# OxfordML/GPz

Measured on AMD Instinct MI355X. Metric: objective+gradient evals/sec, higher is better.
Workload: dtype f64

## Files before the change

### gpz_amd/csrc/gpz_ctx.h

```cpp
#pragma once
#include <hip/hip_runtime.h>
#include <math.h>
#include <stdarg.h>
#include <stdio.h>
#include <stdlib.h>
#include <string.h>
#include <algorithm>
#include <atomic>
#include <mutex>
#include <string>
#include <type_traits>
#include <vector>
#include "../../include/gpz_hip.h"
#include "gpz_dev.h"
#include "gpz_kernels.h"
#include <map>

#define HIPCHK(x)                                                                                   \
    do {                                                                                            \
        hipError_t e_ = (x);                                                                        \
        if (e_ != hipSuccess) return gpz_fail(GPZ_ERR_HIP, "%s:%d %s: %s", __FILE__, __LINE__, #x, hipGetErrorString(e_)); \
    } while (0)

inline int method_id_of(const char *m) {
// ... 173 lines not shown
    int nchunk = 1, rows_per_chunk = 1;
    int tile_rows = 0, ntiles = 1, tile_nchunk = 1, tile_rpc = 1;
    double *tile_rstats = nullptr;
    double *partial = nullptr, *rstats = nullptr, *dGfull = nullptr, *spart = nullptr;
    double *nupart = nullptr, *rowscal = nullptr, *frec = nullptr;
    bool syrk_small = false;
    bool small_tail_dp = false;
    bool small_tail = false;
    int st_nwg = 0, st_nf = 0;
    bool mom_ring = false;
    int mom_nv = 0;
    double *st_slab = nullptr;
    bool fused = true;
    double *phipart = nullptr;
    int phipart_groups = 0;
    long phipart_rows = 0;
    int nslots = 0;
    double *out_d = nullptr;
    double *out_h = nullptr, *theta_h = nullptr;
    gpz_allreduce_fn ar_fn = nullptr;
    void *ar_user = nullptr;
    void *priv = nullptr;
    void (*priv_free)(void *) = nullptr;
    int timing = 0;
    bool time_rest = false;
    struct GraphSeg {
        hipGraphExec_t exec = nullptr;
        int stage = -1;
        bool count_call = false;
        double *hook_buf = nullptr;
// ... 100 lines not shown
```

### gpz_amd/csrc/gpz_ctx.hip

```cpp
#include "gpz_ctx.h"

namespace gpzi {
static int upload_rowset(gpz_ctx *c, RowSet &rs, int64_t n_tot, const double *X, const double *Y, const double *omega,
                         const uint8_t *mask, bool need_xr, const double *Psi = nullptr) {
    const int d = c->d, de = c->de, k = c->k;
    std::vector<int64_t> idx;
    idx.reserve((size_t)n_tot);
    for (int64_t i = 0; i < n_tot; ++i)
        if (!mask || mask[i]) idx.push_back(i);
    if (c->gen) {
        std::vector<int> hg0(idx.size());
        for (size_t r = 0; r < idx.size(); ++r) {
            std::vector<unsigned char> pt(d);
            for (int c_ = 0; c_ < d; ++c_) { const double xv = X[(size_t)c_ * n_tot + idx[r]]; pt[c_] = (xv != xv) ? 0 : 1; }
            int g = -1;
            for (size_t q = 0; q < c->pats.size(); ++q)
                if (c->pats[q] == pt) { g = (int)q; break; }
            if (g < 0) {
                if (c->pats_fixed) return gpz_fail(GPZ_ERR_ARG, "row %lld has a NaN pattern that is not in the given pattern table", (long long)idx[r]);
                c->pats.push_back(pt);
                g = (int)c->pats.size() - 1;
            }
            hg0[r] = g;
        }
// ... 380 lines not shown
        if ((rc = c->ar.alloc(&c->fin_part, (size_t)c->ngroups * c->m * (c->d + c->d * c->d + 2)))) return bail(rc);
        if (!c->has_psi) {
            const int nmt = c->de + c->de * (c->de + 1) / 2;
            c->gen_tnch = 2048 / ((c->m + 255) / 256);
            if (c->gen_tnch < 1) c->gen_tnch = 1;
            if ((rc = build_chunks(c->gen_tnch, 32))) return bail(rc);
            const size_t nslab = c->mom_nchunk > 0 ? (size_t)c->mom_nchunk : 1;
            if ((rc = c->ar.alloc(&c->gen_tslab, nslab * c->m * (nmt + 2)))) return bail(rc);
            if ((rc = c->ar.alloc(&c->gen_frec, (size_t)c->ngroups * c->m * (nmt + 2)))) return bail(rc);
        }
        if (c->va.n_pad && (rc = c->ar.alloc(&c->Phi_v, (size_t)c->va.n_pad * c->mp))) return bail(rc);
    }
    if ((rc = alloc_mm(c))) return bail(rc);

    const size_t np = c->tr.n_pad, mp = c->mp, k = c->k, m = c->m;
    {
        size_t want = c->opt.row_tile > 0 ? (size_t)c->opt.row_tile : 0;
        size_t fr = 0, tot = 0;
        if (!want && hipMemGetInfo(&fr, &tot) == hipSuccess) {
            DevCache &dc = dev_cache();
            std::lock_guard<std::mutex> g(dc.mu);
            auto it = dc.held.find(c->device);
            if (it != dc.held.end()) fr += it->second;
        }
        if (!want && fr && 2.0 * (double)np * (double)mp * 8.0 > 0.7 * (double)fr) {
            want = (size_t)(0.35 * (double)fr / (2.0 * (double)mp * 8.0));
            if (want < 131072) want = 131072;
        }
        const bool can = !c->gen;
        if (want && can) {
            const size_t tr = (size_t)rup((long)want, 1024);
            if (tr < np) {
                c->tile_rows = (int)tr;
                c->ntiles = (int)((np + tr - 1) / tr);
            }
        }
    }
    const size_t npt = c->tile_rows ? (size_t)c->tile_rows : np;
    if ((rc = c->ar.alloc(&c->Phi, npt * mp))) return bail(rc);
    c->small_tail = !c->gen && !c->has_psi && !c->tile_rows &&
                    small_tail_fits(c->kind, c->de, c->m, k, c->mp, c->has_missing) && !c->opt.small_tail_off;
// ... 58 lines not shown
        c->rows_per_split = rup((int)((np_k + s1 - 1) / s1), 16);
        c->nsplit = (int)((np_k + c->rows_per_split - 1) / c->rows_per_split);
        c->rows_per_split_d = rup((int)((np_k + s2 - 1) / s2), 16);
        c->nsplit_d = (int)((np_k + c->rows_per_split_d - 1) / c->rows_per_split_d);
        size_t need = (size_t)(c->nsplit > c->nsplit_d ? c->nsplit : c->nsplit_d) * mp * mp;
        c->syrk_small = syrk_small_fits(mp) && !c->psi32 && !c->opt.syrk_small_off;
        if (c->syrk_small) {
            const size_t ns = syrk_small_slab_count((int)np_k, mp);
            if (ns > need) need = ns;
        }
        size_t need_l = (size_t)c->nsplit_l * c->mq * c->mq;
        c->slab_count = need > need_l ? need : need_l;
        if ((rc = c->ar.alloc(&c->slab, c->slab_count))) return bail(rc);
    }
    {
        size_t prow = npt < 1024 * 1024 ? npt : 0;
        if (c->va.n_pad && (size_t)c->va.n_pad < 1024 * 1024 && (size_t)c->va.n_pad > prow) prow = (size_t)c->va.n_pad;
        if (prow) {
            c->phipart_groups = 16;
            c->phipart_rows = (long)prow;
            if ((rc = c->ar.alloc(&c->phipart, (size_t)c->phipart_groups * 2 * k * prow))) return bail(rc);
        }
    }
    c->comm1_count = k * mp * mp + gpz_ns(c->k);
    if ((rc = c->ar.alloc(&c->comm1, c->comm1_count))) return bail(rc);
    c->comm2_count = m * c->nm + k * 2 * mp + k * 4 + gpz_ns(c->k);
    if ((rc = c->ar.alloc(&c->comm2, c->comm2_count))) return bail(rc);
    c->nwg_rows = c->tr.n < 2048 ? (c->tr.n > 0 ? c->tr.n : 1) : 2048;
    if (!c->fused) {
        if ((rc = c->ar.alloc(&c->colslab, (size_t)c->nwg_rows * 2 * mp))) return bail(rc);
        if ((rc = c->ar.alloc(&c->scal_slab, (size_t)c->nwg_rows * 4))) return bail(rc);
    } else {
        c->nslots = gpz_gemm_wave_cols() * ((c->mp + 127) / 128);
        if ((rc = c->ar.alloc(&c->nupart, (size_t)c->nslots * npt))) return bail(rc);
        if ((rc = c->ar.alloc(&c->rowscal, (size_t)4 * np))) return bail(rc);
        if ((rc = c->ar.alloc(&c->frec, (size_t)m * (c->nm + 2)))) return bail(rc);
// ... 159 lines not shown
    if (f32req && !c->psi32)
        why = !c->gen || !c->has_psi ? " [dtype f32 requested: no input noise on a covariance kind, nothing runs in fp32]"
              : c->d > 20            ? " [dtype f32 requested: d > 20 has no fp32 pair kernel, fp64 route]"
                                     : " [dtype f32 requested: rows with missing dimensions, fp64 route]";
    const int gstate = c->gset[c->timing == 2 ? 1 : 0].state;
    const size_t nseg = c->gset[c->timing == 2 ? 1 : 0].segs.size();
    char gsb[96];
    if (gstate == 2 && nseg > 1) snprintf(gsb, sizeof gsb, "replayed (%zu segments%s)", nseg, c->desc.world > 1 ? ", all-reduce between them" : "");
    else snprintf(gsb, sizeof gsb, "%s", gstate == 2 ? "replayed" : gstate == -1 ? "disabled (recording failed)" : c->opt.no_graph ? "disabled (GPZ_NO_GRAPH)"
                                         : c->timing == 1 ? "off (stage timing on)" : "eager (not recorded yet)");
    const char *gs = gsb;
    const bool f32mm = c->psi32 && !c->opt.f32_contractions_off;
    char rows[96];
    if (c->tile_rows) snprintf(rows, sizeof rows, "; rows: streamed, %d tiles of %d (PHI built twice per evaluation)", c->ntiles, c->tile_rows);
    else rows[0] = 0;
    return snprintf(buf, (size_t)cap, "pair/PHI kernels: %s%s; contractions: %s MFMA%s%s; evaluation graph: %s%s%s", phi, why,
                    f32mm ? "fp32-operand (fp64 master sums)" : "fp64",
                    c->syrk_small ? ", PHI' W PHI with the whole triangle in one workgroup (k_syrk_small)" : "",
                    c->small_tail ? ", T-GEMM + row scalars + moments in one kernel (k_small_tail: T stays in registers)" :
                    c->small_tail_dp ? ", T-GEMM + row scalars + dPHI in one kernel (k_small_tail; moment sums with input noise by k_moments_diag)" : "", gs, rows,
                    c->mom_ring ? "; moments: k_moments_ring (PHI, T through an LDS ring)" : "");
}
namespace gpzi {

}
```

### gpz_amd/csrc/gpz_eval.hip

```cpp
#include "gpz_ctx.h"

namespace gpzi {
static GenRows gen_rows(const RowSet &rs) {
    GenRows r{};
    r.Xr = rs.Xr; r.gid = rs.gid; r.Psi3 = rs.Psi3; r.rows_by_group = rs.rows_by_group; r.n = rs.n; r.n_pad = rs.n_pad;
    return r;
}

static void psi32_chunks(const gpz_ctx *c, int *nch, int *rpc) {
    int r = (c->tr.n + c->gen_nchunk - 1) / c->gen_nchunk;
    r = rup(r > 0 ? r : 1, 64);
    *rpc = r;
    *nch = c->tr.n > 0 ? (c->tr.n + r - 1) / r : 1;
}

static int allreduce(gpz_ctx *c, double *buf, size_t count) {
    if (c->desc.world <= 1) return 0;
    if (!c->ar_fn) return gpz_fail(GPZ_ERR_COMM, "world=%d but no all-reduce hook set (gpz_ctx_set_allreduce)", c->desc.world);
    if (c->capturing) {
        if (graph_cut(c)) return gpz_fail(GPZ_ERR_HIP, "evaluation graph: cut at an exchange point failed");
        c->cap->segs.back().hook_buf = buf;
        c->cap->segs.back().hook_count = count;
        return 0;
    }
// ... 115 lines not shown
            launch_gen_phi(c->st, gen_rows(c->tr), c->m, c->mp, c->d, c->de, c->k, c->pr.P, c->Sig, c->lnS, c->pat_d,
                           c->Phi, c->tr.Y, c->gen_ws);
        }
        launch_gen_rowdot(c->st, c->Phi, c->mp, c->tr.n, c->tr.n_pad, c->m, c->k, c->hetero ? c->pr.v : nullptr, c->pr.b,
                          c->tr.om, nullptr, c->lnbeta, c->wbeta, nullptr, c->tr.om_ld);
    } else {
        Stage s(c, "phi_build");
        PhiArgs a{};
        a.Xc = c->tr.Xc; a.ldx = c->tr.n_pad; a.n = c->tr.n; a.n_pad = c->tr.n_pad;
        a.m = c->m; a.mp = c->mp; a.d = c->de; a.k = c->k; a.kind = c->kind;
        a.P = c->pr.P; a.G = (c->kind == GPZ_KIND_COV) ? c->pr.Rc : c->pr.G2;
        a.v = c->hetero ? c->pr.v : nullptr; a.b = c->pr.b; a.omega = c->tr.om; a.om_ld = c->tr.om_ld; a.Y = c->tr.Y;
        a.Phi = c->Phi; a.lnbeta = c->lnbeta; a.wbeta = c->wbeta; a.w = nullptr; a.phiw = nullptr;
        a.Psic = c->tr.Psic; a.Mc = c->tr.Mc; a.ucnt = c->tr.ucnt;
        a.part = a.n_pad <= c->phipart_rows ? c->phipart : nullptr; a.part_groups = c->phipart_groups;
        if (launch_phi(c->st, a)) return gpz_fail(GPZ_ERR_UNSUPPORTED, "PHI kernel not instantiated for d=%d", c->de);
    }
    return 0;
}

struct RowTile { long r0; int rows, rows_pad; };
static RowTile row_tile(const gpz_ctx *c, int t) {
    RowTile rt;
    rt.r0 = (long)t * c->tile_rows;
    const long left_pad = (long)c->tr.n_pad - rt.r0, left = (long)c->tr.n - rt.r0;
    rt.rows_pad = (int)(left_pad < c->tile_rows ? left_pad : c->tile_rows);
    rt.rows = (int)(left < 0 ? 0 : (left < rt.rows_pad ? left : rt.rows_pad));
    return rt;
}
static int phi_tile(gpz_ctx *c, const RowTile &rt) {
    PhiArgs a{};
    const long r0 = rt.r0;
    a.Xc = c->tr.Xc + r0; a.ldx = c->tr.n_pad; a.n = rt.rows; a.n_pad = rt.rows_pad;
    a.m = c->m; a.mp = c->mp; a.d = c->de; a.k = c->k; a.kind = c->kind;
    a.P = c->pr.P; a.G = (c->kind == GPZ_KIND_COV) ? c->pr.Rc : c->pr.G2;
    a.v = c->hetero ? c->pr.v : nullptr; a.b = c->pr.b; a.omega = c->tr.om ? c->tr.om + r0 : nullptr; a.om_ld = c->tr.om_ld; a.Y = c->tr.Y + r0;
    a.Phi = c->Phi; a.lnbeta = c->lnbeta + r0; a.wbeta = c->wbeta + r0; a.w = nullptr; a.phiw = nullptr;
    a.Psic = c->tr.Psic ? c->tr.Psic + r0 : nullptr; a.Mc = c->tr.Mc ? c->tr.Mc + r0 : nullptr;
    a.ucnt = c->tr.ucnt ? c->tr.ucnt + r0 : nullptr;
    a.part = a.n_pad <= c->phipart_rows ? c->phipart : nullptr; a.part_groups = c->phipart_groups;
    if (launch_phi(c->st, a)) return gpz_fail(GPZ_ERR_UNSUPPORTED, "PHI kernel not instantiated for d=%d", c->de);
    return 0;
}
static int stage_a_tiles(gpz_ctx *c) {
    const bool f32 = c->psi32 && !c->opt.f32_contractions_off;
    for (int t = 0; t < c->ntiles; ++t) {
        const RowTile rt = row_tile(c, t);
        {
            Stage s(c, "phi_build");
            if (int e = phi_tile(c, rt)) return e;
        }
        const int nsp = (rt.rows_pad + c->rows_per_split - 1) / c->rows_per_split;
        const int nsp_d = (rt.rows_pad + c->rows_per_split_d - 1) / c->rows_per_split_d;
        for (int o = 0; o < c->k; ++o) {
            if (c->syrk_small) {
// ... 552 lines not shown
```

### gpz_amd/csrc/gpz_kernels.h

```cpp
#pragma once
#include <hip/hip_runtime.h>
#include <stdint.h>
#include "gpz_options.h"

struct gpz_ctx;
int gpz_fail(int code, const char *fmt, ...);
void gpz_ctx_attach_private(gpz_ctx *c, void *priv, void (*free_fn)(void *));
bool gpz_ctx_allreduce_is(const gpz_ctx *c, int (*fn)(void *, void *, size_t, void *), void **user);
int gpz_ctx_device(const gpz_ctx *c);

struct GpzParams {
    double *P;
    double *G;
    double *G2;
    double *Rc;
    double *lnAlpha;
    double *alpha;
    double *b;
    double *v;
    double *lnTau;
    double *tau;
};

void launch_unpack(hipStream_t st, const double *theta, int method_id, int m, int d, int de, int k, int hetero,
// ... 12 lines not shown
    const double *omega;
    long om_ld;
    const double *Y;
    double *Phi;
    double *lnbeta;
    double *wbeta;
    const double *w;
    double *phiw;
    const double *Psic;
    const double *Mc;
    const double *ucnt;
    double *part;
    int part_groups;
    const int *wgtab;
    int nwg_tab;
};
int phi_cov_rows_per_wg(int de, int k);
bool phi_is_wide(int de, int k);
int phi_wide_rows_per_wg();
int launch_phi_wide(hipStream_t st, const PhiArgs &a);
size_t prep_cov_ws_len(int m, int de);
int launch_prep_cov_wide(hipStream_t st, const double *G, const double *P, int m, int de, double *Rc, double *ws);
void launch_prep_cov(hipStream_t st, const double *G, const double *P, int m, int de, double *Rc, double *ws = nullptr);
int launch_phi(hipStream_t st, const PhiArgs &a);

void launch_syrk(hipStream_t st, const double *Phi, int ld, const double *wgt, int n_rows, int mp,
                 int nsplit, int rows_per_split, int nsplit_d, int rows_per_split_d, double *slab, bool tri,
                 bool f32_operands = false);
bool syrk_small_fits(int mp);
size_t syrk_small_slab_count(int n_rows, int mp);
void launch_syrk_small(hipStream_t st, const double *Phi, int ld, const double *wgt, int n_rows, int mp, double *slab, double *S, int lds,
                       int accumulate);
// ... 370 lines not shown
```

### gpz_amd/csrc/gpz_options.h

```cpp
#pragma once

struct gpz_options {
    bool no_graph = false;
    bool graph_debug = false;
    long row_tile = 0;
    long cache_cap_mb = -1;
    bool psi32_mfma = false;
    long predict_min_rows_per_block = 4096;
    bool f32_contractions_off = false;
    bool gc_minv_off = false;
    bool gc_dense_phi_off = false;
    bool tgemm_no_split = false;
    bool phi_diag_no_split = false;
    bool pmc_scratch = false;
    bool pmc_prep_scratch = false;
    bool pmc_no_model_cache = false;
    bool round_phi32 = false;
    bool cpsi_off = false;
    bool cpsi4_off = false;
    bool tgemm_int8 = false;
    int syrk_wgs = 0, syrk_s1 = 0, syrk_s2 = 0;
    int mom_nc = 0;
    int small_stagger = 0;
    bool chol_rowinv_off = false;
    bool syrk_small_off = false;
    bool small_tail_off = false;
    bool moments_ring_off = false;
    int debug_fail_cut = 0;
};

gpz_options gpz_options_load();

const gpz_options &gpz_opts();
struct gpz_opts_scope {
    const gpz_options *prev;
    explicit gpz_opts_scope(const gpz_options *o);
    ~gpz_opts_scope();
    gpz_opts_scope(const gpz_opts_scope &) = delete;
    gpz_opts_scope &operator=(const gpz_opts_scope &) = delete;
};
```

### gpz_amd/csrc/gpz_options.hip

```cpp
#include <stdlib.h>
#include "gpz_options.h"

static const char *env(const char *name) { return getenv(name); }
static bool env_set(const char *name) { return env(name) != nullptr; }
static long env_long(const char *name, long dflt) {
    const char *e = env(name);
    return e ? atol(e) : dflt;
}

gpz_options gpz_options_load() {
    gpz_options o;
    o.no_graph = env_set("GPZ_NO_GRAPH");
    o.graph_debug = env_set("GPZ_GRAPH_DEBUG");
    o.row_tile = env_long("GPZ_ROW_TILE", 0);
    o.cache_cap_mb = env_long("GPZ_CACHE_CAP_MB", -1);
    {
        const char *e = env("GPZ_PSI32_MFMA");
        o.psi32_mfma = e && e[0] == '1';
    }
    o.predict_min_rows_per_block = env_long("GPZ_PREDICT_MIN_ROWS_PER_BLOCK", 4096);
    if (o.predict_min_rows_per_block < 1) o.predict_min_rows_per_block = 1;
#ifdef GPZ_DEV_SWITCHES
    o.f32_contractions_off = env_set("GPZ_F32_CONTRACTIONS_OFF");
    o.gc_minv_off = env_set("GPZ_GC_MINV_OFF");
// ... 5 lines not shown
    o.pmc_no_model_cache = env_set("GPZ_PMC_NO_MODEL_CACHE");
    o.round_phi32 = env_set("GPZ_EXPERIMENT_ROUND_PHI32");
    o.cpsi_off = env_set("GPZ_CPSI_OFF");
    o.cpsi4_off = env_set("GPZ_CPSI4_OFF");
    o.tgemm_int8 = env_set("GPZ_TGEMM_INT8");
    o.syrk_wgs = (int)env_long("GPZ_SYRK_WGS", 0);
    o.syrk_s1 = (int)env_long("GPZ_SYRK_S1", 0);
    o.syrk_s2 = (int)env_long("GPZ_SYRK_S2", 0);
    o.mom_nc = (int)env_long("GPZ_MOM_NC", 0);
    o.debug_fail_cut = (int)env_long("GPZ_DEBUG_FAIL_CUT", 0);
    o.small_tail_off = env_set("GPZ_SMALL_TAIL_OFF");
    o.syrk_small_off = env_set("GPZ_SYRK_SMALL_OFF");
    o.chol_rowinv_off = env_set("GPZ_CHOL_ROWINV_OFF");
    o.small_stagger = (int)env_long("GPZ_SMALL_STAGGER", 0);
    o.moments_ring_off = env_set("GPZ_MOMENTS_RING_OFF");
#endif
    return o;
}

static thread_local const gpz_options *t_opts = nullptr;
const gpz_options &gpz_opts() {
    if (t_opts) return *t_opts;
    static const gpz_options process = gpz_options_load();
    return process;
}
gpz_opts_scope::gpz_opts_scope(const gpz_options *o) : prev(t_opts) { t_opts = o; }
gpz_opts_scope::~gpz_opts_scope() { t_opts = prev; }
```

### gpz_amd/csrc/k_phi.hip

```cpp
#include <type_traits>
#include "gpz_dev.h"
#include "gpz_kernels.h"

__global__ void k_unpack(const double *__restrict__ theta, int method_id, int m, int d, int de, int k, int hetero,
                         GpzParams pr, int *__restrict__ clear2, double *__restrict__ zero_p, int zero_n) {
    if (clear2 && blockIdx.x == 0 && threadIdx.x < 2) clear2[threadIdx.x] = 0;
    if (zero_p && blockIdx.x == 1)
        for (int e = threadIdx.x; e < zero_n; e += blockDim.x) zero_p[e] = 0.0;
    const int md = m * d;
    int g_dim;
    switch (method_id) {
        case 0: g_dim = 1; break;
        case 1: g_dim = m; break;
        case 2: g_dim = d; break;
        case 3: g_dim = md; break;
        case 4: g_dim = d * d; break;
        default: g_dim = d * d * m; break;
    }
    const int gs = blockDim.x * gridDim.x, t0 = blockIdx.x * blockDim.x + threadIdx.x;
    for (int e = t0; e < m * de; e += gs) {
        const int j = e / de, c = e % de;
        pr.P[e] = (c < d) ? theta[j + m * c] : 0.0;
    }
    if (method_id <= 3) {
// ... 508 lines not shown
        for (int g = 0; g < ngroup; ++g) {
            sv += part[(((size_t)g * 2 + 0) * k + o) * ldp + i];
            sw += part[(((size_t)g * 2 + 1) * k + o) * ldp + i];
        }
        const bool valid = i < n;
        const double lb = bvec[o] + sv;
        lnbeta[(size_t)o * ldx + i] = valid ? lb : 0.0;
        if (wbeta) {
            const double om = omega ? omega[(size_t)o * om_ld + i] : 1.0;
            wbeta[(size_t)o * ldx + i] = valid ? om * exp(-lb) : 0.0;
        }
        if (phiw) phiw[(size_t)o * ldx + i] = valid ? sw : 0.0;
    }
}

static int phi_pick_groups(int nwg, int mp, int JB, int min_wgs, int prologue_cols, int max_groups) {
    const int ncu = gpz_cu_count();
    constexpr int MAXG = 64;
    long cost[MAXG + 1];
    long best_cost = -1;
    if (max_groups > MAXG) max_groups = MAXG;
    if (max_groups < 1) max_groups = 1;
    for (int g = 1; g <= max_groups; ++g) {
        const int jg = ((mp + g - 1) / g + JB - 1) / JB * JB, ge = (mp + jg - 1) / jg;
        cost[g] = -1;
        if (ge != g) continue;
        long per_cu = ((long)nwg * g + ncu - 1) / ncu;
        if (per_cu < min_wgs) per_cu = min_wgs;
        cost[g] = per_cu * (jg + prologue_cols);
        if (best_cost < 0 || cost[g] < best_cost) best_cost = cost[g];
// ... 101 lines not shown
}

bool phi_is_wide(int de, int k) { return de > 20 || k > 8; }
int phi_cov_rows_per_wg(int de, int k) {
    if (phi_is_wide(de, k)) return phi_wide_rows_per_wg();
    switch (de) {
        case 12: return 256 * PhiCovShape<12>::R;
        case 16: return 256 * PhiCovShape<16>::R;
        case 20: return 256 * PhiCovShape<20>::R;
        default: return 256 * PhiCovShape<10>::R;
    }
}

int launch_phi(hipStream_t st, const PhiArgs &a) {
    if (phi_is_wide(a.d, a.k)) return launch_phi_wide(st, a);
    return (a.kind == GPZ_KIND_DIAG) ? launch_phi_k<GPZ_KIND_DIAG>(st, a) : launch_phi_k<GPZ_KIND_COV>(st, a);
}
```

Before: 18.61.

## Add basis-parallel PHI kernel with table-driven exp for small-d COV

Adds k_phi_bases, a PHI kernel for the COV kind with d of 8 or 10 and k=1. Lanes map to basis functions and each lane keeps its Cholesky row in registers, while rows are streamed and the per-row v-weighted sums are reduced through an LDS tile into per-group partials. It replaces libm exp with a 256-entry table exp held in shared memory, enlarges the phipart buffer and changes the row-tiling memory estimate to match. This is meant to cut exp cost and improve parallel mapping, at the price of an extra finalize pass and larger partial buffers.

```diff
diff --git a/gpz_amd/csrc/gpz_ctx.h b/gpz_amd/csrc/gpz_ctx.h
--- a/gpz_amd/csrc/gpz_ctx.h
+++ b/gpz_amd/csrc/gpz_ctx.h
@@ -211,6 +211,7 @@
     bool fused = true;
     double *phipart = nullptr;
     int phipart_groups = 0;
+    bool phi_bases = false;
     long phipart_rows = 0;
     int nslots = 0;
     double *out_d = nullptr;
diff --git a/gpz_amd/csrc/gpz_ctx.hip b/gpz_amd/csrc/gpz_ctx.hip
--- a/gpz_amd/csrc/gpz_ctx.hip
+++ b/gpz_amd/csrc/gpz_ctx.hip
@@ -418,7 +418,9 @@
     if ((rc = alloc_mm(c))) return bail(rc);
 
     const size_t np = c->tr.n_pad, mp = c->mp, k = c->k, m = c->m;
+    c->phi_bases = !c->gen && !c->has_psi && !c->has_missing && c->tr.Xr && phi_bases_fits(c->kind, c->de, c->k) && !c->opt.phi_bases_off;
     {
+        const double row_bytes = 8.0 * (2.0 * (double)mp + (c->phi_bases ? 2.0 * phi_bases_groups((int)mp) * (double)k : 0.0));
         size_t want = c->opt.row_tile > 0 ? (size_t)c->opt.row_tile : 0;
         size_t fr = 0, tot = 0;
         if (!want && hipMemGetInfo(&fr, &tot) == hipSuccess) {
@@ -427,8 +429,8 @@
             auto it = dc.held.find(c->device);
             if (it != dc.held.end()) fr += it->second;
         }
-        if (!want && fr && 2.0 * (double)np * (double)mp * 8.0 > 0.7 * (double)fr) {
-            want = (size_t)(0.35 * (double)fr / (2.0 * (double)mp * 8.0));
+        if (!want && fr && (double)np * row_bytes > 0.7 * (double)fr) {
+            want = (size_t)(0.35 * (double)fr / row_bytes);
             if (want < 131072) want = 131072;
         }
         const bool can = !c->gen;
@@ -517,12 +519,13 @@
         if ((rc = c->ar.alloc(&c->slab, c->slab_count))) return bail(rc);
     }
     {
-        size_t prow = npt < 1024 * 1024 ? npt : 0;
+        size_t prow = npt < 1024 * 1024 || c->phi_bases ? npt : 0;
         if (c->va.n_pad && (size_t)c->va.n_pad < 1024 * 1024 && (size_t)c->va.n_pad > prow) prow = (size_t)c->va.n_pad;
         if (prow) {
             c->phipart_groups = 16;
             c->phipart_rows = (long)prow;
-            if ((rc = c->ar.alloc(&c->phipart, (size_t)c->phipart_groups * 2 * k * prow))) return bail(rc);
+            const size_t groups = c->phi_bases && phi_bases_groups(c->mp) > 16 ? (size_t)phi_bases_groups(c->mp) : 16;
+            if ((rc = c->ar.alloc(&c->phipart, groups * 2 * k * prow))) return bail(rc);
         }
     }
     c->comm1_count = k * mp * mp + gpz_ns(c->k);
@@ -712,13 +715,15 @@
     char rows[96];
     if (c->tile_rows) snprintf(rows, sizeof rows, "; rows: streamed, %d tiles of %d (PHI built twice per evaluation)", c->ntiles, c->tile_rows);
     else rows[0] = 0;
-    return snprintf(buf, (size_t)cap, "pair/PHI kernels: %s%s; contractions: %s MFMA%s%s; evaluation graph: %s%s%s", phi, why,
+    return snprintf(buf, (size_t)cap, "pair/PHI kernels: %s%s; contractions: %s MFMA%s%s; evaluation graph: %s%s%s%s", phi, why,
                     f32mm ? "fp32-operand (fp64 master sums)" : "fp64",
                     c->syrk_small ? ", PHI' W PHI with the whole triangle in one workgroup (k_syrk_small)" : "",
                     c->small_tail ? ", T-GEMM + row scalars + moments in one kernel (k_small_tail: T stays in registers)" :
                     c->small_tail_dp ? ", T-GEMM + row scalars + dPHI in one kernel (k_small_tail; moment sums with input noise by k_moments_diag)" : "", gs, rows,
-                    c->mom_ring ? "; moments: k_moments_ring (PHI, T through an LDS ring)" : "");
-}
-namespace gpzi {
-
-}
+                    c->mom_ring ? "; moments: k_moments_ring (PHI, T through an LDS ring)" : "",
+                    !c->phi_bases ? "" : c->opt.phi_libm_exp ? "; PHI: k_phi_bases (lanes along basis functions, library exp)"
+                                                              : "; PHI: k_phi_bases (lanes along basis functions)");
+}
+namespace gpzi {
+
+}
diff --git a/gpz_amd/csrc/gpz_eval.hip b/gpz_amd/csrc/gpz_eval.hip
--- a/gpz_amd/csrc/gpz_eval.hip
+++ b/gpz_amd/csrc/gpz_eval.hip
@@ -153,6 +153,7 @@
         a.Phi = c->Phi; a.lnbeta = c->lnbeta; a.wbeta = c->wbeta; a.w = nullptr; a.phiw = nullptr;
         a.Psic = c->tr.Psic; a.Mc = c->tr.Mc; a.ucnt = c->tr.ucnt;
         a.part = a.n_pad <= c->phipart_rows ? c->phipart : nullptr; a.part_groups = c->phipart_groups;
+        a.Xr = c->phi_bases ? c->tr.Xr : nullptr;
         if (launch_phi(c->st, a)) return gpz_fail(GPZ_ERR_UNSUPPORTED, "PHI kernel not instantiated for d=%d", c->de);
     }
     return 0;
@@ -178,6 +179,7 @@
     a.Psic = c->tr.Psic ? c->tr.Psic + r0 : nullptr; a.Mc = c->tr.Mc ? c->tr.Mc + r0 : nullptr;
     a.ucnt = c->tr.ucnt ? c->tr.ucnt + r0 : nullptr;
     a.part = a.n_pad <= c->phipart_rows ? c->phipart : nullptr; a.part_groups = c->phipart_groups;
+    a.Xr = c->phi_bases ? c->tr.Xr + (size_t)r0 * c->de : nullptr;
     if (launch_phi(c->st, a)) return gpz_fail(GPZ_ERR_UNSUPPORTED, "PHI kernel not instantiated for d=%d", c->de);
     return 0;
 }
diff --git a/gpz_amd/csrc/gpz_exp.h b/gpz_amd/csrc/gpz_exp.h
--- /dev/null
+++ b/gpz_amd/csrc/gpz_exp.h
@@ -0,0 +1,164 @@
+#pragma once
+#include <math.h>
+#include <stdint.h>
+#include <string.h>
+
+#if defined(__HIPCC__)
+#define GPZ_EXP_HD __host__ __device__
+#else
+#define GPZ_EXP_HD
+#endif
+
+#define GPZ_EXP_TAB_N 256
+#define GPZ_EXP_TABLE { \
+    0x1.0000000000000p+0, 0x0.0p+0, 0x1.00b1afa5abcbfp+0, -0x1.4f6b2a7609f71p-55, \
+    0x1.0163da9fb3335p+0, 0x1.b61299ab8cdb7p-54, 0x1.02168143b0281p+0, -0x1.2bf310fc54eb6p-55, \
+    0x1.02c9a3e778061p+0, -0x1.19083535b085dp-56, 0x1.037d42e11bbccp+0, 0x1.56811eeade11ap-57, \
+    0x1.04315e86e7f85p+0, -0x1.0a31c1977c96ep-54, 0x1.04e5f72f654b1p+0, 0x1.4c3793aa0d08dp-55, \
+    0x1.059b0d3158574p+0, 0x1.d73e2a475b465p-55, 0x1.0650a0e3c1f89p+0, -0x1.5cb7b5799c397p-54, \
+    0x1.0706b29ddf6dep+0, -0x1.c91dfe2b13c27p-55, 0x1.07bd42b72a836p+0, 0x1.3233454458700p-55, \
+    0x1.0874518759bc8p+0, 0x1.186be4bb284ffp-57, 0x1.092bdf66607e0p+0, -0x1.68063800a3fd1p-54, \
+    0x1.09e3ecac6f383p+0, 0x1.1487818316136p-54, 0x1.0a9c79b1f3919p+0, 0x1.5d16c873d1d38p-55, \
+    0x1.0b5586cf9890fp+0, 0x1.8a62e4adc610bp-54, 0x1.0c0f145e46c85p+0, 0x1.4f98906d21cefp-54, \
+    0x1.0cc922b7247f7p+0, 0x1.01edc16e24f71p-54, 0x1.0d83b23395decp+0, -0x1.bc14de43f316ap-54, \
+    0x1.0e3ec32d3d1a2p+0, 0x1.03a1727c57b53p-59, 0x1.0efa55fdfa9c5p+0, -0x1.49db9bc54021bp-54, \
+    0x1.0fb66affed31bp+0, -0x1.b9bedc44ebd7bp-57, 0x1.1073028d7233ep+0, 0x1.d46eb1692fdd5p-55, \
+    0x1.11301d0125b51p+0, -0x1.6c51039449b3ap-54, 0x1.11edbab5e2ab6p+0, -0x1.ca454f703fb72p-54, \
+    0x1.12abdc06c31ccp+0, -0x1.1b514b36ca5c7p-58, 0x1.136a814f204abp+0, -0x1.7108fba48dcf0p-57, \
+    0x1.1429aaea92de0p+0, -0x1.32fbf9af1369ep-54, 0x1.14e95934f312ep+0, -0x1.b91e839bf44abp-55, \
+    0x1.15a98c8a58e51p+0, 0x1.2406ab9eeab0ap-55, 0x1.166a45471c3c2p+0, 0x1.8f23b82ea1a32p-58, \
+    0x1.172b83c7d517bp+0, -0x1.19041b9d78a76p-55, 0x1.17ed48695bbc0p+0, 0x1.09e3fe2ac5a64p-56, \
+    0x1.18af9388c8deap+0, -0x1.11023d1970f6cp-54, 0x1.1972658375d2fp+0, 0x1.4aadd85f17e08p-54, \
+    0x1.1a35beb6fcb75p+0, 0x1.e5b4c7b4968e4p-55, 0x1.1af99f8138a1cp+0, 0x1.7bf85a4b69280p-54, \
+    0x1.1bbe084045cd4p+0, -0x1.95386352ef607p-54, 0x1.1c82f95281c6bp+0, 0x1.009778010f8c9p-54, \
+    0x1.1d4873168b9aap+0, 0x1.e016e00a2643cp-54, 0x1.1e0e75eb44027p+0, -0x1.6fdd8088cb6dep-54, \
+    0x1.1ed5022fcd91dp+0, -0x1.1df98027bb78cp-54, 0x1.1f9c18438ce4dp+0, -0x1.bf524a097af5cp-54, \
+    0x1.2063b88628cd6p+0, 0x1.dc775814a8495p-55, 0x1.212be3578a819p+0, 0x1.3592d2cfcaac9p-54, \
+    0x1.21f49917ddc96p+0, 0x1.2a97e9494a5eep-55, 0x1.22bdda27912d1p+0, 0x1.d34fb5577d69fp-55, \
+    0x1.2387a6e756238p+0, 0x1.9b07eb6c70573p-54, 0x1.2451ffb82140ap+0, 0x1.acfcc911ca996p-55, \
+    0x1.251ce4fb2a63fp+0, 0x1.ac155bef4f4a4p-55, 0x1.25e85711ece75p+0, 0x1.3e1a24ac31b2cp-54, \
+    0x1.26b4565e27cddp+0, 0x1.2bd339940e9d9p-55, 0x1.2780e341ddf29p+0, 0x1.e067c05f9e76cp-54, \
+    0x1.284dfe1f56381p+0, -0x1.a4c3a8c3f0d7ep-54, 0x1.291ba7591bb70p+0, -0x1.2cc7228401cbdp-55, \
+    0x1.29e9df51fdee1p+0, 0x1.612e8afad1255p-55, 0x1.2ab8a66d10f13p+0, -0x1.95743191690a7p-54, \
+    0x1.2b87fd0dad990p+0, -0x1.10adcd6381aa4p-59, 0x1.2c57e39771b2fp+0, -0x1.50145a6eb5124p-54, \
+    0x1.2d285a6e4030bp+0, 0x1.0024754db41d5p-54, 0x1.2df961f641589p+0, 0x1.d16cffbbce198p-54, \
+    0x1.2ecafa93e2f56p+0, 0x1.1ca0f45d52383p-56, 0x1.2f9d24abd886bp+0, -0x1.53c55532bda93p-57, \
+    0x1.306fe0a31b715p+0, 0x1.6f46ad23182e4p-55, 0x1.31432edeeb2fdp+0, 0x1.959a3f3f3fcd1p-55, \
+    0x1.32170fc4cd831p+0, 0x1.a9ce78e18047cp-55, 0x1.32eb83ba8ea32p+0, -0x1.c45e83cb4f318p-54, \
+    0x1.33c08b26416ffp+0, 0x1.32721843659a6p-54, 0x1.3496266e3fa2dp+0, -0x1.35a75930881a4p-55, \
+    0x1.356c55f929ff1p+0, -0x1.b5cee5c4e4628p-55, 0x1.36431a2de883bp+0, -0x1.c3144a06cb85ep-55, \
+    0x1.371a7373aa9cbp+0, -0x1.63aeabf42eae2p-54, 0x1.37f26231e754ap+0, -0x1.9f5ca9eceb23cp-54, \
+    0x1.38cae6d05d866p+0, -0x1.e958d3c9904bdp-54, 0x1.39a401b7140efp+0, -0x1.9a9a5fc8e2934p-54, \
+    0x1.3a7db34e59ff7p+0, -0x1.5e436d661f5e3p-56, 0x1.3b57fbfec6cf4p+0, 0x1.54c66e26fff18p-54, \
+    0x1.3c32dc313a8e5p+0, -0x1.efff8375d29c3p-54, 0x1.3d0e544ede173p+0, 0x1.fe8d08c284c71p-56, \
+    0x1.3dea64c123422p+0, 0x1.ada0911f09ebcp-55, 0x1.3ec70df1c5175p+0, -0x1.af6637b8c9bcap-55, \
+    0x1.3fa4504ac801cp+0, -0x1.7d023f956f9f3p-54, 0x1.40822c367a024p+0, 0x1.bddf8b6f4d048p-55, \
+    0x1.4160a21f72e2ap+0, -0x1.ef3691c309278p-58, 0x1.423fb2709468ap+0, -0x1.8462dc0b314ddp-54, \
+    0x1.431f5d950a897p+0, -0x1.1c7dde35f7999p-55, 0x1.43ffa3f84b9d4p+0, 0x1.880be9704c003p-55, \
+    0x1.44e086061892dp+0, 0x1.89b7a04ef80d0p-59, 0x1.45c2042a7d232p+0, -0x1.8641982fb1f8ep-57, \
+    0x1.46a41ed1d0057p+0, 0x1.c944bd1648a76p-54, 0x1.4786d668b3237p+0, -0x1.c20f0ed445733p-54, \
+    0x1.486a2b5c13cd0p+0, 0x1.3c1a3b69062f0p-56, 0x1.494e1e192aed2p+0, -0x1.3b2895e499ea0p-55, \
+    0x1.4a32af0d7d3dep+0, 0x1.9cb62f3d1be56p-54, 0x1.4b17dea6db7d7p+0, -0x1.125b87f2897f0p-55, \
+    0x1.4bfdad5362a27p+0, 0x1.d4397afec42e2p-56, 0x1.4ce41b817c114p+0, 0x1.05e29690abd5dp-54, \
+    0x1.4dcb299fddd0dp+0, 0x1.8ecdbbc6a7833p-54, 0x1.4eb2d81d8abffp+0, -0x1.5257d2e5d7a52p-54, \
+    0x1.4f9b2769d2ca7p+0, -0x1.4b309d25957e3p-54, 0x1.508417f4531eep+0, 0x1.a249b49b7465fp-56, \
+    0x1.516daa2cf6642p+0, -0x1.f768569bd93efp-55, 0x1.5257de83f4eefp+0, -0x1.c998d43efef71p-56, \
+    0x1.5342b569d4f82p+0, -0x1.07abe1db13cadp-55, 0x1.542e2f4f6ad27p+0, 0x1.7926d192d5f7ep-55, \
+    0x1.551a4ca5d920fp+0, -0x1.d689cefede59bp-55, 0x1.56070dde910d2p+0, -0x1.0fb6e168eebf0p-54, \
+    0x1.56f4736b527dap+0, 0x1.9bb2c011d93adp-54, 0x1.57e27dbe2c4cfp+0, -0x1.0b98c8a57b9c4p-54, \
+    0x1.58d12d497c7fdp+0, 0x1.295e15b9a1de8p-55, 0x1.59c0827ff07ccp+0, -0x1.7e2cee467e60fp-54, \
+    0x1.5ab07dd485429p+0, 0x1.6324c054647adp-54, 0x1.5ba11fba87a03p+0, -0x1.b77a14c233e1ap-54, \
+    0x1.5c9268a5946b7p+0, 0x1.c4b1b816986a2p-60, 0x1.5d84590998b93p+0, -0x1.cd6a7a8b45643p-54, \
+    0x1.5e76f15ad2148p+0, 0x1.ba6f93080e65ep-54, 0x1.5f6a320dceb71p+0, -0x1.9eadde3cdcf92p-55, \
+    0x1.605e1b976dc09p+0, -0x1.3e2429b56de47p-54, 0x1.6152ae6cdf6f4p+0, 0x1.e4b3e4ab84c27p-54, \
+    0x1.6247eb03a5585p+0, -0x1.383c17e40b497p-54, 0x1.633dd1d1929fdp+0, 0x1.84710beb964e5p-54, \
+    0x1.6434634ccc320p+0, -0x1.c483c759d8933p-55, 0x1.652b9febc8fb7p+0, -0x1.ae3d5c9a73e09p-54, \
+    0x1.6623882552225p+0, -0x1.bb60987591c34p-54, 0x1.671c1c70833f6p+0, -0x1.e8732586c6134p-55, \
+    0x1.68155d44ca973p+0, 0x1.038ae44f73e65p-57, 0x1.690f4b19e9538p+0, 0x1.804bd9aeb445dp-55, \
+    0x1.6a09e667f3bcdp+0, -0x1.bdd3413b26456p-54, 0x1.6b052fa75173ep+0, 0x1.a38f52c9a9d0ep-56, \
+    0x1.6c012750bdabfp+0, -0x1.2895667ff0b0dp-56, 0x1.6cfdcddd47645p+0, 0x1.c7aa9b6f17309p-54, \
+    0x1.6dfb23c651a2fp+0, -0x1.bbe3a683c88abp-57, 0x1.6ef9298593ae5p+0, -0x1.0b9749e1ac8b2p-54, \
+    0x1.6ff7df9519484p+0, -0x1.83c0f25860ef6p-55, 0x1.70f7466f42e87p+0, 0x1.9d644d45aa65fp-58, \
+    0x1.71f75e8ec5f74p+0, -0x1.16e4786887a99p-55, 0x1.72f8286ead08ap+0, -0x1.20aa02cd62c72p-54, \
+    0x1.73f9a48a58174p+0, -0x1.0a8d96c65d53cp-54, 0x1.74fbd35d7cbfdp+0, 0x1.047fd618a6e1cp-54, \
+    0x1.75feb564267c9p+0, -0x1.0245957316dd3p-54, 0x1.77024b1ab6e09p+0, 0x1.b7877169147f8p-54, \
+    0x1.780694fde5d3fp+0, 0x1.866b80a02162dp-54, 0x1.790b938ac1cf6p+0, 0x1.349a862aadd3ep-54, \
+    0x1.7a11473eb0187p+0, -0x1.41577ee04992fp-55, 0x1.7b17b0976cfdbp+0, -0x1.bebb58468dc88p-54, \
+    0x1.7c1ed0130c132p+0, 0x1.f124cd1164dd6p-54, 0x1.7d26a62ff86f0p+0, 0x1.1bddbfb72b8b4p-54, \
+    0x1.7e2f336cf4e62p+0, 0x1.05d02ba15797ep-56, 0x1.7f3878491c491p+0, -0x1.07f11cf9311aep-55, \
+    0x1.80427543e1a12p+0, -0x1.27c86626d972bp-54, 0x1.814d2add106d9p+0, 0x1.464370d151d4dp-54, \
+    0x1.82589994cce13p+0, -0x1.d4c1dd41532d8p-54, 0x1.8364c1eb941f7p+0, 0x1.99b9a31df2bd5p-54, \
+    0x1.8471a4623c7adp+0, -0x1.8d684a341cdfbp-55, 0x1.857f4179f5b21p+0, -0x1.ba748f8b216d0p-58, \
+    0x1.868d99b4492edp+0, -0x1.fc6f89bd4f6bap-54, 0x1.879cad931a436p+0, 0x1.5d2d7d2db47bdp-55, \
+    0x1.88ac7d98a6699p+0, 0x1.994c2f37cb53ap-54, 0x1.89bd0a478580fp+0, 0x1.d53954475202bp-54, \
+    0x1.8ace5422aa0dbp+0, 0x1.6e9f156864b27p-54, 0x1.8be05bad61778p+0, 0x1.ecb5efc43446ep-54, \
+    0x1.8cf3216b5448cp+0, -0x1.0d55e32e9e3aap-56, 0x1.8e06a5e0866d9p+0, -0x1.7114a6fc9b2e6p-54, \
+    0x1.8f1ae99157736p+0, 0x1.5cc13a2e3976cp-55, 0x1.902fed0282c8ap+0, 0x1.592ca85fe3fd2p-54, \
+    0x1.9145b0b91ffc6p+0, -0x1.dd6792e582524p-54, 0x1.925c353aa2fe2p+0, -0x1.3455fa639db7fp-55, \
+    0x1.93737b0cdc5e5p+0, -0x1.75fc781b57ebcp-57, 0x1.948b82b5f98e5p+0, -0x1.dc3d6797d2d99p-55, \
+    0x1.95a44cbc8520fp+0, -0x1.64b7c96a5f039p-56, 0x1.96bdd9a7670b3p+0, -0x1.ba5967f19c896p-58, \
+    0x1.97d829fde4e50p+0, -0x1.d185b7c1b85d1p-54, 0x1.98f33e47a22a2p+0, 0x1.cabdaa24c78edp-56, \
+    0x1.9a0f170ca07bap+0, -0x1.173bd91cee632p-54, 0x1.9b2bb4d53fe0dp+0, -0x1.dd84e4df6d518p-54, \
+    0x1.9c49182a3f090p+0, 0x1.c7c46b071f2bep-56, 0x1.9d674194bb8d5p+0, -0x1.516bea3dd8233p-54, \
+    0x1.9e86319e32323p+0, 0x1.824ca78e64c6ep-56, 0x1.9fa5e8d07f29ep+0, -0x1.4a9ceaaf1facep-55, \
+    0x1.a0c667b5de565p+0, -0x1.359495d1cd533p-54, 0x1.a1e7aed8eb8bbp+0, 0x1.c6618ee8be70ep-54, \
+    0x1.a309bec4a2d33p+0, 0x1.6305c7ddc36abp-54, 0x1.a42c980460ad8p+0, -0x1.aa780589fb120p-54, \
+    0x1.a5503b23e255dp+0, -0x1.d2f6edb8d41e1p-54, 0x1.a674a8af46052p+0, 0x1.50f5630670366p-57, \
+    0x1.a799e1330b358p+0, 0x1.bcb7ecac563c7p-54, 0x1.a8bfe53c12e59p+0, -0x1.4f867b2ba15a9p-54, \
+    0x1.a9e6b5579fdbfp+0, 0x1.0fac90ef7fd31p-54, 0x1.ab0e521356ebap+0, 0x1.89c31dae94545p-55, \
+    0x1.ac36bbfd3f37ap+0, -0x1.f9234cae76cd0p-55, 0x1.ad5ff3a3c2774p+0, 0x1.7ef3bb6b1b8e5p-54, \
+    0x1.ae89f995ad3adp+0, 0x1.7a1cd345dcc81p-54, 0x1.afb4ce622f2ffp+0, -0x1.4b2fc0f315ecdp-54, \
+    0x1.b0e07298db666p+0, -0x1.bdef54c80e425p-54, 0x1.b20ce6c9a8952p+0, 0x1.4dd024a0756ccp-54, \
+    0x1.b33a2b84f15fbp+0, -0x1.2805e3084d708p-57, 0x1.b468415b749b1p+0, -0x1.f763de9df7c90p-56, \
+    0x1.b59728de5593ap+0, -0x1.c71dfbbba6de3p-54, 0x1.b6c6e29f1c52ap+0, 0x1.2a8f352883f6ep-54, \
+    0x1.b7f76f2fb5e47p+0, -0x1.5584f7e54ac3bp-56, 0x1.b928cf22749e4p+0, -0x1.b721654cb65c6p-54, \
+    0x1.ba5b030a1064ap+0, -0x1.efcd30e54292ep-54, 0x1.bb8e0b79a6f1fp+0, -0x1.f52d1c9696205p-60, \
+    0x1.bcc1e904bc1d2p+0, 0x1.23dd07a2d9e84p-55, 0x1.bdf69c3f3a207p+0, -0x1.c262360ea5b52p-60, \
+    0x1.bf2c25bd71e09p+0, -0x1.efdca3f6b9c73p-54, 0x1.c06286141b33dp+0, -0x1.d8a5aa1fbca34p-55, \
+    0x1.c199bdd85529cp+0, 0x1.11065895048ddp-55, 0x1.c2d1cd9fa652cp+0, -0x1.6e51617c8a5d7p-54, \
+    0x1.c40ab5fffd07ap+0, 0x1.b4537e083c60ap-54, 0x1.c544778fafb22p+0, 0x1.12f072493b5afp-54, \
+    0x1.c67f12e57d14bp+0, 0x1.2884dff483cadp-54, 0x1.c7ba88988c933p+0, -0x1.e76bbbe255559p-55, \
+    0x1.c8f6d9406e7b5p+0, 0x1.1acbc48805c44p-56, 0x1.ca3405751c4dbp+0, -0x1.7f2bed10d08f5p-55, \
+    0x1.cb720dcef9069p+0, 0x1.503cbd1e949dbp-56, 0x1.ccb0f2e6d1675p+0, -0x1.d220f86009093p-56, \
+    0x1.cdf0b555dc3fap+0, -0x1.dd83b53829d72p-55, 0x1.cf3155b5bab74p+0, -0x1.a08e9b86dff57p-54, \
+    0x1.d072d4a07897cp+0, -0x1.cbc3743797a9cp-54, 0x1.d1b532b08c968p+0, 0x1.55636219a36eep-54, \
+    0x1.d2f87080d89f2p+0, -0x1.d487b719d8578p-54, 0x1.d43c8eacaa1d6p+0, 0x1.3db53bf5a1614p-54, \
+    0x1.d5818dcfba487p+0, 0x1.2ed02d75b3707p-55, 0x1.d6c76e862e6d3p+0, 0x1.fe87a4a8165a0p-58, \
+    0x1.d80e316c98398p+0, -0x1.11ec18beddfe8p-54, 0x1.d955d71ff6075p+0, 0x1.a052dbb9af6bep-54, \
+    0x1.da9e603db3285p+0, 0x1.c2300696db532p-54, 0x1.dbe7cd63a8315p+0, -0x1.b76f1926b8be4p-54, \
+    0x1.dd321f301b460p+0, 0x1.2da5778f018c3p-54, 0x1.de7d5641c0658p+0, -0x1.ca5528e79ba8fp-54, \
+    0x1.dfc97337b9b5fp+0, -0x1.1a5cd4f184b5cp-54, 0x1.e11676b197d17p+0, -0x1.2b529bd5c7f44p-56, \
+    0x1.e264614f5a129p+0, -0x1.7b627817a1496p-54, 0x1.e3b333b16ee12p+0, -0x1.9f4a431fdc68bp-54, \
+    0x1.e502ee78b3ff6p+0, 0x1.39e8980a9cc8fp-55, 0x1.e653924676d76p+0, -0x1.63ff87522b735p-55, \
+    0x1.e7a51fbc74c83p+0, 0x1.2d522ca0c8de2p-54, 0x1.e8f7977cdb740p+0, -0x1.1089480b054b1p-54, \
+    0x1.ea4afa2a490dap+0, -0x1.e9c23179c2893p-54, 0x1.eb9f4867cca6ep+0, 0x1.4832f2293e4f2p-54, \
+    0x1.ecf482d8e67f1p+0, -0x1.c93f3b411ad8cp-54, 0x1.ee4aaa2188510p+0, 0x1.1c68da487568dp-54, \
+    0x1.efa1bee615a27p+0, 0x1.dc7f486a4b6b0p-54, 0x1.f0f9c1cb6412ap+0, -0x1.3220065181d45p-54, \
+    0x1.f252b376bba97p+0, 0x1.3a1a5bf0d8e43p-54, 0x1.f3ac948dd7274p+0, -0x1.95a5a3ed837dep-56, \
+    0x1.f50765b6e4540p+0, 0x1.9d3e12dd8a18bp-54, 0x1.f6632798844f8p+0, 0x1.fa37b3539343ep-54, \
+    0x1.f7bfdad9cbe14p+0, -0x1.dbb12d006350ap-54, 0x1.f91d802243c89p+0, -0x1.12ea8a779f689p-57, \
+    0x1.fa7c1819e90d8p+0, 0x1.74853f3a5931ep-55, 0x1.fbdba3692d514p+0, -0x1.9677315098eb6p-56, \
+    0x1.fd3c22b8f71f1p+0, 0x1.2eb74966579e7p-57, 0x1.fe9d96b2a23d9p+0, 0x1.4a6037442fde3p-56, \
+}
+
+GPZ_EXP_HD inline double gpz_exp_nhalf(double q, const double *tab) {
+    uint64_t b;
+    memcpy(&b, &q, sizeof b);
+    const uint32_t hi = q > 2048.0 ? 0x40A00000u : (uint32_t)(b >> 32);
+    b = ((uint64_t)hi << 32) | (b & 0xffffffffull);
+    memcpy(&q, &b, sizeof q);
+    const double t = fma(q, -0x1.71547652b82fep+7, 0x1.8p+52);
+    const double kd = t - 0x1.8p+52;
+    uint64_t tb;
+    memcpy(&tb, &t, sizeof tb);
+    const int k = (int)(uint32_t)tb;
+    double u = fma(kd, 0x1.62e42fefa39efp-8, q);
+    u = fma(kd, 0x1.abc9e3b39803fp-63, u);
+    double p = fma(u, 0x1.5555555555555p-9, -0x1.5555555555555p-6);
+    p = fma(p, u, 0.125);
+    p = fma(p, u, -0.5);
+    p *= u;
+    const unsigned off = ((unsigned)k << 4) & (unsigned)(16 * GPZ_EXP_TAB_N - 16);
+    const double th = *(const double *)((const char *)tab + off), tl = *(const double *)((const char *)tab + off + 8);
+    return ldexp(th + fma(th, p, tl), k >> 8);
+}
diff --git a/gpz_amd/csrc/gpz_kernels.h b/gpz_amd/csrc/gpz_kernels.h
--- a/gpz_amd/csrc/gpz_kernels.h
+++ b/gpz_amd/csrc/gpz_kernels.h
@@ -50,8 +50,11 @@
     int part_groups;
     const int *wgtab;
     int nwg_tab;
+    const double *Xr;
 };
 int phi_cov_rows_per_wg(int de, int k);
+bool phi_bases_fits(int kind, int de, int k);
+int phi_bases_groups(int mp);
 bool phi_is_wide(int de, int k);
 int phi_wide_rows_per_wg();
 int launch_phi_wide(hipStream_t st, const PhiArgs &a);
diff --git a/gpz_amd/csrc/gpz_options.h b/gpz_amd/csrc/gpz_options.h
--- a/gpz_amd/csrc/gpz_options.h
+++ b/gpz_amd/csrc/gpz_options.h
@@ -26,6 +26,8 @@
     bool syrk_small_off = false;
     bool small_tail_off = false;
     bool moments_ring_off = false;
+    bool phi_bases_off = false;
+    bool phi_libm_exp = false;
     int debug_fail_cut = 0;
 };
 
diff --git a/gpz_amd/csrc/gpz_options.hip b/gpz_amd/csrc/gpz_options.hip
--- a/gpz_amd/csrc/gpz_options.hip
+++ b/gpz_amd/csrc/gpz_options.hip
@@ -43,6 +43,8 @@
     o.chol_rowinv_off = env_set("GPZ_CHOL_ROWINV_OFF");
     o.small_stagger = (int)env_long("GPZ_SMALL_STAGGER", 0);
     o.moments_ring_off = env_set("GPZ_MOMENTS_RING_OFF");
+    o.phi_bases_off = env_set("GPZ_PHI_BASES_OFF");
+    o.phi_libm_exp = env_set("GPZ_PHI_LIBM_EXP");
 #endif
     return o;
 }
diff --git a/gpz_amd/csrc/k_phi.hip b/gpz_amd/csrc/k_phi.hip
--- a/gpz_amd/csrc/k_phi.hip
+++ b/gpz_amd/csrc/k_phi.hip
@@ -1,5 +1,6 @@
 #include <type_traits>
 #include "gpz_dev.h"
+#include "gpz_exp.h"
 #include "gpz_kernels.h"
 
 __global__ void k_unpack(const double *__restrict__ theta, int method_id, int m, int d, int de, int k, int hetero,
@@ -546,6 +547,126 @@
     }
 }
 
+#define PB_RB 4
+#define PB_FL 32
+#define PB_LD 66
+template <int D, bool HASV, bool LIBM>
+__global__ __launch_bounds__(128) void k_phi_bases(const double *__restrict__ Xr, int n, int n_pad, int m, int mp, int ngroup,
+                                                   int rows_per_chunk, const double *__restrict__ Rc, const double *__restrict__ v,
+                                                   const double *__restrict__ Y, double *__restrict__ Phi, double *__restrict__ part,
+                                                   long ldp) {
+    constexpr int NT = D * (D + 1) / 2, NP = NT + D;
+    static constexpr double tab_init[2 * GPZ_EXP_TAB_N] = GPZ_EXP_TABLE;
+    __shared__ __align__(16) double etab[2 * GPZ_EXP_TAB_N];
+    __shared__ __align__(16) double red[2][PB_FL * PB_LD];
+    const int tid = threadIdx.x, lane = tid & 63;
+    const int wave = __builtin_amdgcn_readfirstlane(tid >> 6);
+    if (!LIBM) {
+        for (int e = tid; e < 2 * GPZ_EXP_TAB_N; e += 128) etab[e] = tab_init[e];
+        __syncthreads();
+    }
+    const int g = blockIdx.x * 2 + wave;
+    if (g >= ngroup) return;
+    const int j0 = g * 64, j = j0 + lane;
+    const int r0 = blockIdx.y * rows_per_chunk, r1 = min(n_pad, r0 + rows_per_chunk);
+    const int rfull = max(r0, min(r1, n / PB_FL * PB_FL));
+    double rj[NP];
+#pragma unroll
+    for (int e = 0; e < NP; ++e) rj[e] = j < m ? Rc[(size_t)j * NP + e] : 0.0;
+    const double vj = (HASV && j < m) ? v[j] : 0.0;
+    double *tile = red[wave];
+    double *pg = part + (size_t)g * 2 * ldp;
+    unsigned loff = (unsigned)lane * 8u;
+
+    auto rows = [&](auto edge_c, auto tail_c, int i, int tb) {
+        constexpr bool EDGE = decltype(edge_c)::value, TAIL = decltype(tail_c)::value;
+        double x[PB_RB][D];
+#pragma unroll
+        for (int r = 0; r < PB_RB; ++r)
+#pragma unroll
+            for (int c = 0; c < D; ++c) x[r][c] = Xr[(size_t)(i + r) * D + c];
+        double q[PB_RB];
+#pragma unroll
+        for (int r = 0; r < PB_RB; ++r) q[r] = 0.0;
+#pragma unroll
+        for (int a = 0; a < D; ++a) {
+            const int ro = a * D - a * (a - 1) / 2;
+            double s[PB_RB];
+#pragma unroll
+            for (int r = 0; r < PB_RB; ++r) s[r] = fma(rj[ro], x[r][a], -rj[NT + a]);
+#pragma unroll
+            for (int b = a + 1; b < D; ++b)
+#pragma unroll
+                for (int r = 0; r < PB_RB; ++r) s[r] = fma(rj[ro + b - a], x[r][b], s[r]);
+#pragma unroll
+            for (int r = 0; r < PB_RB; ++r) q[r] = fma(s[r], s[r], q[r]);
+        }
+#pragma unroll
+        for (int r = 0; r < PB_RB; ++r) {
+            double ph = LIBM ? exp(-0.5 * q[r]) : gpz_exp_nhalf(q[r], etab);
+            if (TAIL) ph = (i + r < n) ? ph : 0.0;
+            if (HASV) tile[(tb + r) * PB_LD + lane] = ph * vj;
+            asm volatile("" : "+v"(loff));
+            double *prow = reinterpret_cast<double *>(reinterpret_cast<char *>(Phi + ((size_t)(i + r) * mp + j0)) + loff);
+            if (EDGE) {
+                const double y = Y ? Y[i + r] : 0.0;
+                ph = j < m ? ph : (j == m ? y : 0.0);
+                if (j < mp) *prow = ph;
+            } else {
+                *prow = ph;
+            }
+        }
+    };
+    auto flush = [&](int i0) {
+        __builtin_amdgcn_wave_barrier();
+        const int rr = lane & 31, h = lane >> 5;
+        const double *src = tile + rr * PB_LD + 32 * h;
+        double a0 = src[0], a1 = src[1], a2 = src[2], a3 = src[3];
+#pragma unroll
+        for (int c = 4; c < 32; c += 4) { a0 += src[c]; a1 += src[c + 1]; a2 += src[c + 2]; a3 += src[c + 3]; }
+        double acc = (a0 + a1) + (a2 + a3);
+        acc += __shfl_xor(acc, 32, 64);
+        asm volatile("" : "+v"(loff));
+        if (lane < 32) *reinterpret_cast<double *>(reinterpret_cast<char *>(pg + i0) + loff) = acc;
+        __builtin_amdgcn_wave_barrier();
+    };
+    auto walk = [&](auto edge_c) {
+        for (int i0 = r0; i0 < rfull; i0 += PB_FL) {
+#pragma unroll 1
+            for (int tb = 0; tb < PB_FL; tb += PB_RB) rows(edge_c, std::false_type{}, i0 + tb, tb);
+            if (HASV) flush(i0);
+        }
+        for (int i0 = rfull; i0 < r1; i0 += PB_FL) {
+#pragma unroll 1
+            for (int tb = 0; tb < PB_FL; tb += PB_RB) rows(edge_c, std::true_type{}, i0 + tb, tb);
+            if (HASV) flush(i0);
+        }
+    };
+    if (j0 + 64 <= m) walk(std::false_type{});
+    else walk(std::true_type{});
+}
+
+bool phi_bases_fits(int kind, int de, int k) { return kind == GPZ_KIND_COV && (de == 8 || de == 10) && k == 1; }
+int phi_bases_groups(int mp) { return (mp + 63) / 64; }
+
+template <int D>
+static void launch_phi_bases_d(hipStream_t st, const PhiArgs &a) {
+    const int ngroup = phi_bases_groups(a.mp), wgx = (ngroup + 1) / 2;
+    long nch = (4L * gpz_cu_count() + wgx - 1) / wgx;
+    const int rpc = (int)(((a.n_pad + nch - 1) / nch + PB_FL - 1) / PB_FL * PB_FL);
+    nch = (a.n_pad + rpc - 1) / rpc;
+    const bool hasv = a.v != nullptr, libm = gpz_opts().phi_libm_exp;
+    const dim3 grid((unsigned)wgx, (unsigned)nch);
+#define PHI_BASES(HV, LM) \
+    hipLaunchKernelGGL((k_phi_bases<D, HV, LM>), grid, dim3(128), 0, st, a.Xr, a.n, a.n_pad, a.m, a.mp, ngroup, rpc, a.G, a.v, a.Y, \
+                       a.Phi, a.part, (long)a.n_pad)
+    if (hasv) { if (libm) PHI_BASES(true, true); else PHI_BASES(true, false); }
+    else { if (libm) PHI_BASES(false, true); else PHI_BASES(false, false); }
+#undef PHI_BASES
+    hipLaunchKernelGGL(k_phi_finalize, dim3((unsigned)((a.n_pad + 255) / 256)), dim3(256), 0, st, (const double *)a.part, (long)a.n_pad,
+                       hasv ? ngroup : 0, a.ldx, (long)a.n_pad, a.n, a.k, a.b, a.omega, a.om_ld, a.lnbeta, a.wbeta, a.phiw);
+}
+
 static int phi_pick_groups(int nwg, int mp, int JB, int min_wgs, int prologue_cols, int max_groups) {
     const int ncu = gpz_cu_count();
     constexpr int MAXG = 64;
@@ -677,5 +798,10 @@
 
 int launch_phi(hipStream_t st, const PhiArgs &a) {
     if (phi_is_wide(a.d, a.k)) return launch_phi_wide(st, a);
+    if (a.Xr && a.Phi && a.part && !a.wgtab && !a.w && !a.phiw && phi_bases_fits(a.kind, a.d, a.k)) {
+        if (a.d == 8) launch_phi_bases_d<8>(st, a);
+        else launch_phi_bases_d<10>(st, a);
+        return 0;
+    }
     return (a.kind == GPZ_KIND_DIAG) ? launch_phi_k<GPZ_KIND_DIAG>(st, a) : launch_phi_k<GPZ_KIND_COV>(st, a);
 }
```

Result: slower. 18.00 (-3.3%).
